# georgegrosu1/torch-admm-deconv

Hardware: AMD Instinct MI355X
Metric: ADMM iterations/sec, batch-64 1024x1024x3, 50 iters; rel-L2 vs CPU ref (higher is better)
Workload: dtype f32

## Files before the change

### torch-admm-deconv_amd/csrc/admm_capi.hip

```cpp
#include <hip/hip_runtime.h>

#include <cstdlib>
#include <cstring>
#include <mutex>
#include <string>
#include <type_traits>
#include <vector>

#include "gcol_mm.hpp"
#include "knobs.hpp"
#include "mixed_capi.hpp"
#include "odd_capi.hpp"
#include "state_kernels.hpp"
#include "admm_tv.h"

using namespace admm;

namespace {

thread_local std::string g_err;

int fail(int code, const std::string& msg) {
    g_err = msg;
    return code;
// ... 88 lines not shown
    size_t lds;
    int nth;
};
MMPlan mm_plan(int H, int W);
MMPlan mm_plan_row(int W);

int ngroups_of(const admm_tv_desc& d) { return d.groups > 1 ? d.groups : 1; }

bool is_bank(const admm_tv_desc& d) { return (d.flags & (ADMM_TV_FLAG_PSF_PER_IMAGE | ADMM_TV_FLAG_PSF_PER_CHANNEL)) != 0; }
BankIdx bank_of(const admm_tv_desc& d) {
    const int Bk = (d.flags & ADMM_TV_FLAG_PSF_PER_IMAGE) ? (int)d.B : 1;
    const int Ck = (d.flags & ADMM_TV_FLAG_PSF_PER_CHANNEL) ? (int)d.C : 1;
    return BankIdx{(int)d.C, Bk > 1 ? Ck : 0, Ck > 1 ? 1 : 0, Bk * Ck};
}
int bank_run(const admm_tv_desc& d) { return (d.flags & ADMM_TV_FLAG_PSF_PER_CHANNEL) ? 1 : (int)d.C; }
constexpr long long kBankMax = 65535;

constexpr size_t kAlign = 256;
size_t up(size_t v) { return (v + kAlign - 1) / kAlign * kAlign; }

struct Layout {
    size_t spec[2], u[4], b, fcT, mT, twW, twH, twHd, G, part, nsq, sigma, total;
    size_t mM;
    MMPlan mm, mmr;
    bool mixed, mixed_train;
    size_t fcM;
    bool odd;
    size_t spec2;
    bool tr;
    size_t xT, oT, kT, tws;
    size_t rimg;
    size_t gscr;
    int ngroups, ppg;
    bool gen;
    int ldw;
};

admm_tv_desc transposed(const admm_tv_desc& d) {
    admm_tv_desc t = d;
    t.H = d.W;
    t.W = d.H;
    t.kh = d.kw;
    t.kw = d.kh;
    return t;
}

// ... 15 lines not shown
    size_t o = 0;
    auto take = [&](size_t bytes) {
        size_t at = o;
        o += up(bytes);
        return at;
    };
    L.gen = f64 || generic_hw(d.H, d.W);
    if (L.gen && !f64) {
        if (!bank) L.mm = mm_plan((int)H, (int)W);
        L.mmr = mm_plan_row((int)W);
    }
    L.mixed = L.gen && !f64 && mixed_hw(d.H, d.W) && (G == 1 || !(d.flags & ADMM_TV_FLAG_PSF_GRAD));
    L.mixed_train = mixed_train_hw(d);
    L.odd = L.gen && !f64 && G == 1 && !d.iso && !bank && odd_hw(d.H, d.W);
    L.ldw = (int)(N + 1);
    if (L.gen && !f64 && L.mm.ok && L.mmr.ok && env_int("ADMM_GEN_PITCH", 1)) L.ldw = (int)((N + 1 + 15) / 16 * 16);
    L.spec[0] = take(L.gen ? P * H * (size_t)L.ldw * csz : img);
    L.spec[1] = take(img);
    L.rimg = L.gen ? take(img) : 0;
    for (int i = 0; i < 4; ++i) L.u[i] = take(img);
    L.b = (k > 0 || !L.gen) ? take(img_m) : 0;
    L.fcT = take(G * T * (N + 1) * H * rs * ((!L.gen || L.mm.ok) ? 2 : 1));
    L.mT = take(T * (N + 1) * H * csz);
    L.twW = take((W + (L.gen ? make_plan((int)W, f64).ntab : 0)) * csz);
    L.twH = take((H + (L.gen ? make_plan((int)H, f64).ntab : 0)) * csz);
    L.twHd = take(H * sizeof(double2));
    L.G = take(T * (size_t)(k > 0 ? k : 1) * (N + 1) * sizeof(double2));
    L.gscr = L.gen ? take(glb_scratch((int)H, (int)W, (long long)P, f64)) : 0;
    L.fcM = L.mixed ? take(G * T * (2 * N + 1) * H * sizeof(float)) : 0;
    L.mM = (L.mixed && k > 0) ? take(T * (N + 1) * H * 2 * sizeof(float)) : 0;
    L.spec2 = L.odd ? take(P * H * (size_t)L.ldw * csz) : 0;
    L.sigma = (k > 0 && (d.flags & ADMM_TV_FLAG_PSF_GRAD)) ? take((N + 1) * H * sizeof(double2)) : 0;
    if (d.iso) {
        const int lanes = (int)std::min<size_t>(64, N / (N >= 1024 ? 16 : N >= 64 ? 8 : N >= 16 ? 4 : 2));
        const long long want = 3LL * 1024 * 64 / std::max(lanes, 1);
        int ppg = (int)std::max<long long>(1, std::min<long long>(64, (long long)(P * H) / want));
        if (const int e = env_int("ADMM_ISO_PPG", 0); e > 0) ppg = e;
        if ((size_t)P <= (size_t)ppg) ppg = (int)std::max<long long>(1, P);
        if (G > 1) {
            const int pm = (int)(d.B * d.C);
            ppg = std::min(ppg, pm);
            while (pm % ppg) --ppg;
        }
        L.ppg = ppg;
        L.ngroups = (int)((P + ppg - 1) / ppg);
        L.part = take((size_t)L.ngroups * 2 * H * W * rs);
// ... 46 lines not shown
}

int check_workspace(const void* ws, size_t have, size_t need) {
    if (!ws || have < need || (reinterpret_cast<uintptr_t>(ws) % kAlign) != 0)
        return fail(ADMM_TV_EWORKSPACE, "workspace too small or not 256-byte aligned");
    return 0;
}

template <class T>
int bwd_scalars(double* part, int K, long long nstrips, long long spm, long long soff, const double* tpart, int ntp,
                int G, int g, const T* lam, const T* rho, T* glam, T* grho, hipStream_t s) {
    if (K < 1) return fail(ADMM_TV_EINVAL, "bwd_scalars: no iterations");
    hipLaunchKernelGGL(k_bwd_iter_sums, dim3((unsigned)K), dim3(256), 0, s, part, nstrips, spm, soff, tpart, ntp, G, g);
    if (int e = launch_check("k_bwd_iter_sums")) return e;
    hipLaunchKernelGGL(k_bwd_scalars<T>, dim3(1), dim3(256), 0, s, (const double*)part, K, nstrips, 1LL, soff,
                       (const double*)nullptr, ntp, G, g, lam, rho, glam, grho);
    return launch_check("k_bwd_scalars");
}

template <int N> struct RowOps {
    using G = RowKernelGeom<N>;
    static unsigned blocks(long long items) { return (unsigned)((items + G::SG - 1) / G::SG); }

    static int r2c(const float* img, cf* spec, const cf* twW, long long rows, hipStream_t s, bool pl = false) {
        if (pl)
            hipLaunchKernelGGL((k_row_r2c<N, true>), dim3(blocks(rows)), dim3(G::NT), G::lds_bytes(), s, img, spec, twW, rows);
        else
            hipLaunchKernelGGL((k_row_r2c<N, false>), dim3(blocks(rows)), dim3(G::NT), G::lds_bytes(), s, img, spec, twW, rows);
        return launch_check("k_row_r2c");
    }
    static int c2r(const cf* spec, float* img, const cf* twW, long long rows, hipStream_t s, bool pl = false) {
        if (pl)
            hipLaunchKernelGGL((k_row_c2r<N, true>), dim3(blocks(rows)), dim3(G::NT), G::lds_bytes(), s, spec, img, twW, rows);
        else
            hipLaunchKernelGGL((k_row_c2r<N, false>), dim3(blocks(rows)), dim3(G::NT), G::lds_bytes(), s, spec, img, twW, rows);
        return launch_check("k_row_c2r");
    }
    static int pair(const float* img, float* out, long long rows, hipStream_t s) {
        hipLaunchKernelGGL(k_row_pair<N>, dim3(blocks(rows)), dim3(G::NT), 0, s, img, out, rows);
        return launch_check("k_row_pair");
    }
    template <bool ISO, bool FIRST, bool HIST, bool PL> static void pa(const PassAArgs& a, unsigned nb, hipStream_t s) {
        hipLaunchKernelGGL((k_pass_a<N, ISO, FIRST, HIST, PL>), dim3(nb), dim3(G::NT), G::lds_bytes(), s, a);
    }
    static constexpr bool kCoop = N == 512;
    template <bool FIRST, bool PL> static void pa_coop(const PassAArgs& a, unsigned nb, hipStream_t s, bool pf) {
        if constexpr (kCoop) {
            if (pf)
                hipLaunchKernelGGL((k_pass_a<N, false, FIRST, false, PL, true, true>), dim3(nb), dim3(G::NT), passa_coop_lds<N>(), s, a);
            else
                hipLaunchKernelGGL((k_pass_a<N, false, FIRST, false, PL, true>), dim3(nb), dim3(G::NT), passa_coop_lds<N>(), s, a);
        }
    }
    static int pass_a(const PassAArgs& a, bool iso, bool first, bool hist, hipStream_t s, bool pl = false,
                      bool coop = false, bool pf = false) {
// ... 94 lines not shown
        case 256: return f(std::integral_constant<int, 256>{});
        case 512: return f(std::integral_constant<int, 512>{});
        case 1024: return f(std::integral_constant<int, 1024>{});
        case 2048: return f(std::integral_constant<int, 2048>{});
        case 4096: return f(std::integral_constant<int, 4096>{});
        default: return fail(ADMM_TV_EUNSUPPORTED, "unsupported H");
    }
}

int col_e(int H) { return H >= 1024 ? 16 : H >= 64 ? 8 : 4; }

int passb_order(int H) { return std::max(1, std::min(64, env_int("ADMM_PASSB_GROUP", H >= 1024 ? 2 : 1))); }

int passb_gp(int H, int P, int ppm) {
    (void)H;
    int g = env_int("ADMM_PASSB_GP", 1);
    g = std::max(1, std::min(g, 64));
    while (g > 1 && (ppm % g)) --g;
    (void)P;
    return g;
}

template <int H, int C> int pass_b_hc(const cf* spec, cf* out, const float* fcT, const cf* mT, const cf* twH, int N,
                                      int P, int mode, int ppm, hipStream_t s, const BankIdx* bank) {
    using G = ColGeom<H, C>;
    const int colblocks = N / C;
    const int gp = passb_gp(H, P, ppm);
    const dim3 grid((unsigned)((long long)((P + gp - 1) / gp) * colblocks));
    const int order = gp > 1 ? 1 : passb_order(H);
    const int fpack = mode == 0 && env_int("ADMM_PASSB_FPACK", 1) ? 1 : 0;
    const int pmode = env_int("ADMM_PASSB_PMODE", 2);
    if (bank) {
        if (mode == 0) {
            if (int e = set_lds(k_pass_b<H, C, 0, BankIdx>, G::lds_bytes())) return e;
            hipLaunchKernelGGL((k_pass_b<H, C, 0, BankIdx>), grid, dim3(G::NT), G::lds_bytes(), s, spec, out, fcT, mT, twH, N,
                               colblocks, ppm, order, fpack, gp, P, pmode, *bank);
        } else if (mode == 1) {
            if (int e = set_lds(k_pass_b<H, C, 1, BankIdx>, G::lds_bytes())) return e;
            hipLaunchKernelGGL((k_pass_b<H, C, 1, BankIdx>), grid, dim3(G::NT), G::lds_bytes(), s, spec, out, fcT, mT, twH, N,
                               colblocks, ppm, order, fpack, gp, P, pmode, *bank);
        } else {
            return fail(ADMM_TV_EUNSUPPORTED, "PSF bank: no adjoint column pass (inference only)");
        }
        return launch_check("k_pass_b<bank>");
    }
    if (mode == 0) {
        if (int e = set_lds(k_pass_b<H, C, 0>, G::lds_bytes())) return e;
        hipLaunchKernelGGL((k_pass_b<H, C, 0>), grid, dim3(G::NT), G::lds_bytes(), s, spec, out, fcT, mT, twH, N, colblocks, ppm,
                           order, fpack, gp, P, pmode);
    } else if (mode == 1) {
        if (int e = set_lds(k_pass_b<H, C, 1>, G::lds_bytes())) return e;
        hipLaunchKernelGGL((k_pass_b<H, C, 1>), grid, dim3(G::NT), G::lds_bytes(), s, spec, out, fcT, mT, twH, N, colblocks, ppm,
                           order, fpack, gp, P, pmode);
    } else {
        if (int e = set_lds(k_pass_b<H, C, 2>, G::lds_bytes())) return e;
        hipLaunchKernelGGL((k_pass_b<H, C, 2>), grid, dim3(G::NT), G::lds_bytes(), s, spec, out, fcT, mT, twH, N, colblocks, ppm,
                           order, fpack, gp, P, pmode);
    }
    return launch_check("k_pass_b");
}

template <int H> int pass_b_h(const cf* spec, cf* out, const float* fcT, const cf* mT, const cf* twH, int N, int P,
                              int mode, int ppm, hipStream_t s, const BankIdx* bank) {
    constexpr int L = ColGeom<H, 1>::L;
    if constexpr (L <= 64) {
        if (mode == 0 && N >= 16 && env_int("ADMM_PASSB_PAIR", H <= 512 ? 1 : 0)) {
            using G = ColGeom<H, 8>;
            const int colblocks = N / 16;
            if (bank) {
                if (int e = set_lds(k_pass_b2<H, 8, BankIdx>, G::lds_bytes())) return e;
                hipLaunchKernelGGL((k_pass_b2<H, 8, BankIdx>), dim3((unsigned)((long long)P * colblocks)), dim3(G::NT),
                                   G::lds_bytes(), s, spec, out, fcT, twH, N, colblocks, ppm, passb_order(H),
                                   env_int("ADMM_PASSB_FPACK", 1) ? 1 : 0, *bank);
                return launch_check("k_pass_b2<bank>");
            }
            if (int e = set_lds(k_pass_b2<H, 8>, G::lds_bytes())) return e;
            hipLaunchKernelGGL((k_pass_b2<H, 8>), dim3((unsigned)((long long)P * colblocks)), dim3(G::NT), G::lds_bytes(),
                               s, spec, out, fcT, twH, N, colblocks, ppm, passb_order(H), env_int("ADMM_PASSB_FPACK", 1) ? 1 : 0);
            return launch_check("k_pass_b2");
        }
        int C = env_int("ADMM_PASSB_C", 8);
        if (C > N) C = N;
        if (C >= 16) return pass_b_hc<H, 16>(spec, out, fcT, mT, twH, N, P, mode, ppm, s, bank);
        return pass_b_hc<H, 8>(spec, out, fcT, mT, twH, N, P, mode, ppm, s, bank);
    } else if constexpr (L == 128) {
        return pass_b_hc<H, 8>(spec, out, fcT, mT, twH, N, P, mode, ppm, s, bank);
    } else {
        return pass_b_hc<H, 4>(spec, out, fcT, mT, twH, N, P, mode, ppm, s, bank);
    }
}

int pass_b_oop(int H, const cf* spec, cf* out, const float* fcT, const cf* mT, const cf* twH, int N, int P, int mode,
               hipStream_t s, int ppm = 0, const BankIdx* bank = nullptr) {
    if (ppm <= 0) ppm = P;
    return with_col(H, [&](auto h) { return pass_b_h<decltype(h)::value>(spec, out, fcT, mT, twH, N, P, mode, ppm, s, bank); });
}

int pass_b(int H, cf* spec, const float* fcT, const cf* mT, const cf* twH, int N, int P, int mode, hipStream_t s,
           int ppm = 0, const BankIdx* bank = nullptr) {
    return pass_b_oop(H, spec, spec, fcT, mT, twH, N, P, mode, s, ppm, bank);
}

template <int H, int C> int xspec_hc(const cf* U, const cf* V, cf* part, const cf* twH, int N, int P, int ppg,
                                     hipStream_t s) {
    using G = ColGeom<H, C>;
    const int colblocks = N / C;
    const int groups = (P + ppg - 1) / ppg;
    if (int e = set_lds(k_xspec<H, C, true>, G::lds_bytes())) return e;
    if (int e = set_lds(k_xspec<H, C, false>, G::lds_bytes())) return e;
    hipLaunchKernelGGL((k_xspec<H, C, true>), dim3(groups), dim3(G::NT), G::lds_bytes(), s, U, V, part, twH, N,
                       colblocks, P, ppg);
    if (colblocks > 1)
        hipLaunchKernelGGL((k_xspec<H, C, false>), dim3(groups * (colblocks - 1)), dim3(G::NT), G::lds_bytes(), s, U,
                           V, part, twH, N, colblocks, P, ppg);
    return launch_check("k_xspec");
}
template <int H> int xspec_h(const cf* U, const cf* V, cf* part, const cf* twH, int N, int P, int ppg, hipStream_t s) {
    constexpr int L = ColGeom<H, 1>::L;
    if constexpr (L <= 64) return xspec_hc<H, 8>(U, V, part, twH, N, P, ppg, s);
    else if constexpr (L == 128) return xspec_hc<H, 8>(U, V, part, twH, N, P, ppg, s);
    else return xspec_hc<H, 4>(U, V, part, twH, N, P, ppg, s);
}
int xspec(int H, const cf* U, const cf* V, cf* part, const cf* twH, int N, int P, int ppg, hipStream_t s) {
// ... 20 lines not shown
    if (d->groups > 1 && ((!supported_hw(d->H, d->W) && !mixed_hw(d->H, d->W)) || (d->flags & ADMM_TV_FLAG_PSF_GRAD)))
        return fail(ADMM_TV_EUNSUPPORTED, "groups > 1 needs power-of-two or smooth H, W and no PSF gradient");
    return 0;
}

int bank_check(const admm_tv_desc& d, bool train = false, bool f64 = false) {
    if (!is_bank(d)) return 0;
    if (f64 || is_f64(d)) return fail(ADMM_TV_EUNSUPPORTED, "PSF bank: fp32 only (ADMM_TV_FLAG_F64 / an _f64 entry point)");
    if (train) return fail(ADMM_TV_EUNSUPPORTED, "PSF bank: inference only (training with a bank is not implemented)");
    if (d.flags & ADMM_TV_FLAG_PSF_GRAD) return fail(ADMM_TV_EUNSUPPORTED, "PSF bank: no PSF gradient (ADMM_TV_FLAG_PSF_GRAD)");
    if (d.kh == 0) return fail(ADMM_TV_EINVAL, "PSF bank without a PSF (kh == 0)");
    if (d.groups > 1) return fail(ADMM_TV_EUNSUPPORTED, "PSF bank: groups > 1 (one solve per module)");
    if (d.allreduce) return fail(ADMM_TV_EUNSUPPORTED, "PSF bank: no cross-rank all-reduce hook");
    const long long T = ((d.flags & ADMM_TV_FLAG_PSF_PER_IMAGE) ? d.B : 1) * ((d.flags & ADMM_TV_FLAG_PSF_PER_CHANNEL) ? d.C : 1);
    if (T > kBankMax || d.B > 0x7fffffffLL || d.C > 0x7fffffffLL)
        return fail(ADMM_TV_EUNSUPPORTED, "PSF bank: more than 65,535 PSFs");
    return 0;
}

double spectra_scale(int H, int W) {
    return (supported_hw(H, W) ? 0.5 : 1.0) / ((double)H * (double)W);
}

int bank_spectra(const admm_tv_desc& d, const Layout& Lo, void* ws, const float* rho, float* fcT, hipStream_t s) {
    const int H = (int)d.H, W = (int)d.W, N = W / 2, nt = 256, n = (N + 1) * H;
    const unsigned T = (unsigned)bank_of(d).T;
    hipLaunchKernelGGL(k_spectra_bank, dim3((n + nt - 1) / nt, T), dim3(nt), 0, s, at<double2>(ws, Lo.G),
                       at<double2>(ws, Lo.twHd), rho, fcT, at<cf>(ws, Lo.mT), d.kh, H, N, W, spectra_scale(H, W));
    if (int e = launch_check("k_spectra_bank")) return e;
    if (Lo.mixed) return hip_code(admm_mixed::mt_mixed(at<cf>(ws, Lo.mT), at<cf>(ws, Lo.mM), H, N, s, (int)T), "k_mt_mixed_bank");
    return 0;
}
int setup_bank(const admm_tv_desc& d, const Layout& Lo, void* ws, const float* kern, const float* rho, hipStream_t s) {
    const int H = (int)d.H, W = (int)d.W, N = W / 2, k = d.kh, nt = 256, n = (N + 1) * H;
    const unsigned T = (unsigned)bank_of(d).T;
    hipLaunchKernelGGL(k_psf_rows_bank, dim3((k * (N + 1) + nt - 1) / nt, T), dim3(nt), 0, s, kern, at<double2>(ws, Lo.G), k,
                       N, W);
    if (int e = launch_check("k_psf_rows_bank")) return e;
    if (!rho) return 0;
    float* fc = at<float>(ws, Lo.fcT);
    if (int e = bank_spectra(d, Lo, ws, rho, fc, s)) return e;
    if (!Lo.gen) {
        hipLaunchKernelGGL(k_fc_pack_bank, dim3((n + nt - 1) / nt, T), dim3(nt), 0, s, fc, fc + (size_t)T * n, H, N, col_e(H));
        if (int e = launch_check("k_fc_pack_bank")) return e;
    }
    if (Lo.mixed) return hip_code(admm_mixed::fc_mixed(fc, at<float>(ws, Lo.fcM), H, N, s, (int)T), "k_fc_mixed_bank");
    return 0;
}

template <class T>
int setup(const admm_tv_desc& d, const Layout& Lo, void* ws, const T* kern, const T* rho, hipStream_t s) {
    using C = cx_t<T>;
// ... 27 lines not shown
                               at<double2>(ws, Lo.twHd), rho + g, at<T>(ws, Lo.fcT) + (size_t)g * n, at<C>(ws, Lo.mT),
                               k, H, N, W, Lo.sigma ? at<double2>(ws, Lo.sigma) : nullptr,
                               (std::is_same<T, double>::value ? 1.0 / ((double)H * W) : spectra_scale(H, W)));
            if (int e = launch_check("k_spectra")) return e;
            if constexpr (std::is_same<T, float>::value) if (!Lo.gen) {
                float* fc = at<float>(ws, Lo.fcT) + (size_t)g * n;
                hipLaunchKernelGGL(k_fc_pack, dim3((n + nt - 1) / nt), dim3(nt), 0, s, fc,
                                   fc + (size_t)ngroups_of(d) * n, H, N, col_e(H));
                if (int e = launch_check("k_fc_pack")) return e;
            }
            if constexpr (std::is_same<T, float>::value) if (Lo.mixed) {
                if (int e = hip_code(admm_mixed::fc_mixed(at<float>(ws, Lo.fcT) + (size_t)g * n,
                                                          at<float>(ws, Lo.fcM) + (size_t)g * (2 * N + 1) * H, H, N, s),
                                     "k_fc_mixed"))
                    return e;
            }
            if constexpr (std::is_same<T, float>::value) if (Lo.gen && Lo.mm.ok && ngroups_of(d) == 1) {
                float* fc = at<float>(ws, Lo.fcT);
                hipLaunchKernelGGL(k_fc_transpose, dim3(std::min(4096, (n + nt - 1) / nt)), dim3(nt), 0, s, fc, fc + n, H,
                                   N + 1);
                if (int e = launch_check("k_fc_transpose")) return e;
            }
        }
        if constexpr (std::is_same<T, float>::value) if (Lo.mixed && k > 0) {
            if (int e = hip_code(admm_mixed::mt_mixed(at<cf>(ws, Lo.mT), at<cf>(ws, Lo.mM), H, N, s), "k_mt_mixed")) return e;
        }
    }
    return 0;
}

int pow2_floor(int v);

int strip_rows(int H, int N, long long rows, bool aniso_fwd = false, bool coop = false) {
    int R = env_int("ADMM_PASSA_R", 0);
    if (R > 0) R = pow2_floor(std::max(2, std::min(R, H)));
    if (R <= 0) {
        const int L = std::min(64, N / (N >= 1024 ? 16 : N >= 64 ? 8 : N >= 16 ? 4 : 2));
        long long want = 3LL * 1024 * 64 / L;
        R = 8;
        if (aniso_fwd && N == 256) {
            R = 16;
            want /= 2;
        }
        if (coop && aniso_fwd && N == 512 && (H / 4) % 4 == 0) R = 4;
        while (R > 2 && rows / R < want) R /= 2;
    }
// ... 78 lines not shown
            hipError_t e = hipEventRecord(joins[i], aux[i]);
            if (e == hipSuccess) e = hipStreamWaitEvent(s, joins[i], 0);
            if (first == hipSuccess) first = e;
        }
        return first;
    }
    ~ForkJoin() {
        if (fork) (void)hipEventDestroy(fork);
        for (hipEvent_t j : joins)
            if (j) (void)hipEventDestroy(j);
    }
};

std::vector<long long> gen_parts(long long P, int H, int ns) {
    long long c = (P + ns - 1) / std::max(ns, 1);
    if (H & 1) c += c & 1;
    std::vector<long long> starts;
    for (long long p = 0; p < P; p += std::max(c, 1LL)) starts.push_back(p);
    return starts;
}


int psf_transpose_into(const admm_tv_desc& d, const Layout& Lo, void* ws, const float* xin, float* bb, cf* spec,
                       int mode, hipStream_t s, bool pl = false) {
    const long long rows = d.B * d.C * d.H;
    const int H = (int)d.H, N = (int)d.W / 2;
    cf* twW = at<cf>(ws, Lo.twW);
    int e = with_row(N, [&](auto ops) { return decltype(ops)::r2c(xin, spec, twW, rows, s); });
    if (e) return e;
    const BankIdx bk = bank_of(d);
    if ((e = pass_b(H, spec, at<float>(ws, Lo.fcT), at<cf>(ws, Lo.mT), at<cf>(ws, Lo.twH), N, (int)(d.B * d.C), mode, s,
                    is_bank(d) ? bank_run(d) : 0, is_bank(d) ? &bk : nullptr)))
        return e;
    return with_row(N, [&](auto ops) { return decltype(ops)::c2r(spec, bb, twW, rows, s, pl); });
}


GPlan make_plan_radices(int n);

int blue_min() { return env_int("ADMM_BLUE_MIN", 41); }

constexpr size_t kMaxLds = 160 * 1024;
size_t glds(int n, int lines, const GPlan& p, size_t csz = sizeof(cf)) {
    if (p.glb) return 0;
    return csz * ((p.twg ? 0 : (size_t)n + p.ntab) + 2 * (size_t)n * lines + p.xslots);
}

constexpr long long kGlbSlots = 1024;
constexpr size_t kGlbBudget = 512ull << 20;
long long glb_slots(int n, size_t csz) {
    return std::max<long long>(64, std::min<long long>(kGlbSlots, (long long)(kGlbBudget / (2 * (size_t)n * csz))));
}

GPlan make_plan_f64(int n) {
    GPlan p{};
    p.n = n;
    int m = n, r = n;
// ... 853 lines not shown
    FusedOps(const admm_tv_desc& d_, const Layout& L, void* w)
        : d(d_), Lo(L), ws(w), H((int)d_.H), N((int)d_.W / 2), twW(at<cf>(w, L.twW)), twH(at<cf>(w, L.twH)) {}
};

struct Pow2Ops : FusedOps {
    static constexpr bool kPsfGrad = true;
    float* const fcT;
    cf* const mT;
    const bool coop;
    const int rev;
    const bool pf;
    Pow2Ops(const admm_tv_desc& d_, const Layout& L, void* w)
        : FusedOps(d_, L, w), fcT(at<float>(w, L.fcT)), mT(at<cf>(w, L.mT)),
          coop(env_int("ADMM_PASSA_COOP", 1) != 0), rev(env_int("ADMM_PASSA_REV", 0)),
          pf(env_int("ADMM_PASSA_PF", 1) != 0) {}
    int modules_per_pass(int G) const { return G; }
    bool lane_paired(bool train) const { return !train && env_int("ADMM_PL", (d.iso || d.W < 1024) ? 1 : 0) != 0; }
    int row_lanes() const {
        int L = 0;
        with_row(N, [&](auto ops) { return L = decltype(ops)::G::L; });
        return L;
    }
    int strip(long long rows, bool aniso_fwd) const { return strip_rows(H, N, rows, aniso_fwd, coop && !rev); }
    int r2c(const float* img, cf* spec, long long rows, hipStream_t s, bool pl = false) const {
        return with_row(N, [&](auto ops) { return decltype(ops)::r2c(img, spec, twW, rows, s, pl); });
    }
    int c2r(const cf* spec, float* img, long long rows, hipStream_t s) const {
        return with_row(N, [&](auto ops) { return decltype(ops)::c2r(spec, img, twW, rows, s); });
    }
    int col(const cf* in, cf* out, long long np, long long ppm, int , hipStream_t s) const {
        if (is_bank(d)) {
            const BankIdx bk = bank_of(d);
            return pass_b_oop(H, in, out, fcT, mT, twH, N, (int)np, 0, s, bank_run(d), &bk);
        }
        return pass_b_oop(H, in, out, fcT, mT, twH, N, (int)np, 0, s, (int)ppm);
    }
    int xspec(const cf* U, const cf* V, cf* part, long long P, int ppg, bool , hipStream_t s) const {
        return ::xspec(H, U, V, part, twH, N, (int)P, ppg, s);
    }
    int iso_norm(const IsoArgs& a, bool first, bool hist, hipStream_t s, bool pl) const {
        return with_row(N, [&](auto ops) { return decltype(ops)::iso_norm(a, first, hist, s, pl); });
    }
    int pass_a(const PassAArgs& a, bool iso, bool first, bool hist, hipStream_t s, bool pl) const {
        return with_row(N, [&](auto ops) { return decltype(ops)::pass_a(a, iso, first, hist, s, pl, coop, pf); });
    }
    int bwd_iso_q(const BwdIsoArgs& a, bool lastk, hipStream_t s) const {
        return with_row(N, [&](auto ops) { return decltype(ops)::bwd_iso_q(a, lastk, s); });
    }
    int bwd_pass_a(const BwdArgs& a, bool iso, bool lastk, bool firstk, hipStream_t s) const {
        return with_row(N, [&](auto ops) { return decltype(ops)::bwd_pass_a(a, iso, lastk, firstk, s); });
    }
    int make_b(const float* xin, float* bb, cf* spec, bool pl, hipStream_t s) const {
        if (d.kh > 0) return psf_transpose_into(d, Lo, ws, xin, bb, spec, 1, s, pl);
        return with_row(N, [&](auto ops) { return decltype(ops)::pair(xin, bb, d.B * d.C * H, s); });
    }
    int apply_ht_t(const float* bbar, float* gxin, cf* spec, hipStream_t s) const {
        return psf_transpose_into(d, Lo, ws, bbar, gxin, spec, 2, s);
    }
};

struct MixedOps : FusedOps {
    static constexpr bool kPsfGrad = true;
    const float* const fcM;
    static constexpr int rev = 0;
    MixedOps(const admm_tv_desc& d_, const Layout& L, void* w) : FusedOps(d_, L, w), fcM(at<float>(w, L.fcM)) {}
    int modules_per_pass(int) const { return 1; }
    bool lane_paired(bool) const { return false; }
    int row_lanes() const { return 0; }
    int strip(long long rows, bool) const { return strip_rows_mixed(H, rows, N); }
    int r2c(const float* img, cf* spec, long long rows, hipStream_t s, bool = false) const {
        return hip_code(admm_mixed::r2c(N, img, spec, twW, rows, s), "k_row_r2c_m");
    }
    int c2r(const cf* spec, float* img, long long rows, hipStream_t s) const {
        return hip_code(admm_mixed::c2r(N, spec, img, twW, rows, s), "k_row_c2r_m");
    }
    int col(const cf* in, cf* out, long long np, long long, int g0, hipStream_t s) const {
        if (is_bank(d)) {
            const BankIdx bk = bank_of(d);
            return hip_code(admm_mixed::pass_b(H, in, out, fcM, twH, N, np, s, &bk), "k_pass_b_m<bank>");
        }
        return hip_code(admm_mixed::pass_b(H, in, out, fcM + (size_t)g0 * (2 * N + 1) * H, twH, N, np, s), "k_pass_b_m");
    }
    int xspec(const cf* U, const cf* V, cf* part, long long P, int ppg, bool weighted, hipStream_t s) const {
        return hip_code(admm_mixed::xspec(H, U, V, part, twH, N, P, ppg, weighted ? 0.25f : 1.f, s), "k_xspec_m");
    }
    int iso_norm(const IsoArgs& a, bool first, bool hist, hipStream_t s, bool) const {
        return hip_code(admm_mixed::iso_norm(N, a, first, hist, s), "k_iso_norm_m");
    }
    int pass_a(const PassAArgs& a, bool iso, bool first, bool hist, hipStream_t s, bool) const {
        return hip_code(admm_mixed::pass_a(N, a, iso, first, hist, s), "k_pass_a_m");
    }
    int bwd_iso_q(const BwdIsoArgs& a, bool lastk, hipStream_t s) const {
        return hip_code(admm_mixed::bwd_iso_q(N, a, lastk, s), "k_bwd_iso_q_m");
    }
    int bwd_pass_a(const BwdArgs& a, bool iso, bool lastk, bool firstk, hipStream_t s) const {
        return hip_code(admm_mixed::bwd_pass_a(N, a, iso, lastk, firstk, s), "k_bwd_pass_a_m");
    }
    int make_b(const float* xin, float* bb, cf* spec, bool, hipStream_t s) const {
        const long long P = d.B * d.C;
        if (env_int("ADMM_MIXED_BGEN", 0)) return gapply<float>(xin, bb, spec, Lo, ws, d, 1, s);
        if (int e = r2c(xin, spec, P * H, s)) return e;
        const BankIdx bk = bank_of(d);
        if (int e = hip_code(admm_mixed::pass_b_cm(H, spec, at<cf>(ws, Lo.mM), twH, N, P, s, is_bank(d) ? &bk : nullptr),
                             "k_pass_b_m<cm>"))
            return e;
        return c2r(spec, bb, P * H, s);
    }
    int apply_ht_t(const float* bbar, float* gxin, cf* spec, hipStream_t s) const {
        return gapply<float>(bbar, gxin, spec, Lo, ws, d, 2, s);
    }
};

template <class B>
int fused_forward(const B& be, const float* xin, const float* lam, const float* rho, float* out, void* hist,
                  hipStream_t s, const StateIO* sio = nullptr) {
    const admm_tv_desc& d = be.d;
    const Layout& Lo = be.Lo;
    void* ws = be.ws;
    const int H = be.H, N = be.N, W = (int)d.W, G = ngroups_of(d);
    const long long Pm = d.B * d.C;
    cf* spec[2] = {at<cf>(ws, Lo.spec[0]), at<cf>(ws, Lo.spec[1])};
    float* u[4] = {at<float>(ws, Lo.u[0]), at<float>(ws, Lo.u[1]), at<float>(ws, Lo.u[2]), at<float>(ws, Lo.u[3])};
    const bool train = hist != nullptr;
    const HistView<float> hv(d, hist);
    const bool keep_t = B::kPsfGrad && train && hv.h.keep_t;
    const bool pl = be.lane_paired(train);
    const float* bimg = xin;
    if (d.kh > 0 || pl) {
        ProfScope ps(3, s);
        float* bb = at<float>(ws, Lo.b);
        if (int e = be.make_b(xin, bb, spec[0], pl, s)) return e;
        bimg = bb;
    }
    const int ng = be.modules_per_pass(G);
    const long long np = ng * Pm, rows = np * H;
    const int gpm = Lo.ngroups / G;
    const int R = be.strip(rows, !d.iso && !train);
    const bool sin = sio && sio->in, sout = sio && sio->out;
    const int sl = pl ? be.row_lanes() : 0;
    for (int g0 = 0; g0 < G; g0 += ng) {
        const float* lamg = lam + g0;
        const float* rhog = rho + g0;
        float* outg = out + (size_t)g0 * Pm * H * W;
        for (int g = 0; g < ng; ++g) {
            ProfScope ps(3, s);
            cf* t0 = (keep_t ? hv.r(1) : spec[0]) + (size_t)g * Pm * H * N;
            if (sin) {
                if (int e = state_import(d, *sio->in, bimg, outg, u[0], u[1], lamg, rhog, sl, s)) return e;
                if (int e = be.r2c(outg, t0, Pm * H, s, false)) return e;
                continue;
            }
            if (int e = be.r2c(bimg, t0, Pm * H, s, pl)) return e;
        }
        int cur = 0, uin = 0;
        for (int it = 1; it <= d.maxit; ++it) {
            {
                ProfScope ps(1, s);
                if (int e = be.col(keep_t ? hv.r(it) : spec[cur], spec[cur], np, Pm, g0, s)) return e;
            }
            if (it == d.maxit) {
                ProfScope ps(3, s);
                if (int e = be.c2r(spec[cur], outg, rows, s)) return e;
                if (sout) {
                    const bool none = d.maxit == 1 && !sin;
                    if (int e = state_export(d, Lo, ws, outg, none ? nullptr : u[2 * uin], none ? nullptr : u[2 * uin + 1],
                                             *sio->out, lamg, rhog, sl, s))
                        return e;
                }
                if (!train) break;
// ... 599 lines not shown
    DeviceGuard dg(reinterpret_cast<hipStream_t>(stream));
    if (int e = dg.check()) return e;
    const Layout Lo = make_layout(d);
    if (!ws || ws_bytes < Lo.total) return fail(ADMM_TV_EWORKSPACE, "workspace too small");
    const long long P = d.B * d.C;
    const int H = (int)d.H, W = (int)d.W, N = W / 2;
    if (d.kh == 0) {
        HIPCHK(hipMemcpyAsync(out, xin, (size_t)P * H * W * sizeof(float), hipMemcpyDeviceToDevice, s));
        return 0;
    }
    if (int e = setup<float>(d, Lo, ws, kern, nullptr, s)) return e;
    const int n = (N + 1) * H;
    HIPCHK(hipMemsetAsync(at<float>(ws, Lo.fcT), 0, sizeof(float), s));
    if (is_bank(d)) {
        if (int e = bank_spectra(d, Lo, ws, at<float>(ws, Lo.fcT), at<float>(ws, Lo.spec[1]), s)) return e;
        if (Lo.mixed) return MixedOps(d, Lo, ws).make_b(xin, out, at<cf>(ws, Lo.spec[0]), false, s);
        if (Lo.gen) return gapply(xin, out, at<cf>(ws, Lo.spec[0]), Lo, ws, d, 1, s);
        return psf_transpose_into(d, Lo, ws, xin, out, at<cf>(ws, Lo.spec[0]), 1, s);
    }
    hipLaunchKernelGGL(k_spectra<float>, dim3((n + 255) / 256), dim3(256), 0, s, at<double2>(ws, Lo.G),
                       at<double2>(ws, Lo.twHd), at<float>(ws, Lo.fcT), at<float>(ws, Lo.spec[1]),
                       at<cf>(ws, Lo.mT), d.kh, H, N, W, nullptr, spectra_scale(H, W));
    if (int e = launch_check("k_spectra")) return e;
    if (Lo.gen) return gapply(xin, out, at<cf>(ws, Lo.spec[0]), Lo, ws, d, 1, s);
    return psf_transpose_into(d, Lo, ws, xin, out, at<cf>(ws, Lo.spec[0]), 1, s);
}

int admm_tv_forward_f64(const admm_tv_desc* dp, const double* xin, const double* kern, const double* lam,
                        const double* rho, double* out, void* ws, size_t ws_bytes, void* stream) {
    if (int e = validate(dp)) return e;
    if (int e = bank_check(*dp, false, true)) return e;
    if (!is_f64(*dp)) return fail(ADMM_TV_EINVAL, "admm_tv_forward_f64 needs ADMM_TV_FLAG_F64");
    if (((!xin || !out) && !participate_only(*dp)) || !lam || !rho || (dp->kh > 0 && !kern))
        return fail(ADMM_TV_EINVAL, "null pointer argument");
    DeviceGuard dg(reinterpret_cast<hipStream_t>(stream));
    if (int e = dg.check()) return e;
    return run_forward_f64(*dp, xin, kern, lam, rho, out, ws, ws_bytes, nullptr, reinterpret_cast<hipStream_t>(stream));
}

int admm_tv_forward_train_f64(const admm_tv_desc* dp, const double* xin, const double* kern, const double* lam,
                              const double* rho, double* out, void* hist, size_t hist_bytes, void* ws, size_t ws_bytes,
                              void* stream) {
    if (int e = validate(dp)) return e;
    if (int e = bank_check(*dp, false, true)) return e;
    if (!is_f64(*dp)) return fail(ADMM_TV_EINVAL, "admm_tv_forward_train_f64 needs ADMM_TV_FLAG_F64");
    if (((!xin || !out) && !participate_only(*dp)) || !lam || !rho || (dp->kh > 0 && !kern))
// ... 66 lines not shown
```

### torch-admm-deconv_amd/csrc/admm_kernels.hpp

```cpp
#pragma once
#include "fft_core.hpp"

namespace admm {

template <int N, class Cfg = RowCfg<N>> struct RowXf {
    static constexpr int E = Cfg::E;
    static constexpr int L = N / E;
    static constexpr int W = 2 * N;
    static_assert(L <= 64, "row transforms keep one row inside one wave");

    __device__ __forceinline__ static void partner(const cf (&v)[E], cf (&p)[E], int t) {
        const int src = (L - t) & (L - 1);
#pragma unroll
        for (int j = 0; j < E; ++j) {
            float a = __shfl(v[E - 1 - j].x, src, L);
            float b = __shfl(v[E - 1 - j].y, src, L);
            p[j] = (t == 0) ? v[(E - j) & (E - 1)] : mkc(a, b);
        }
    }

    template <int SYNC = 0>
    __device__ __forceinline__ static void c2r(cf (&v)[E], const RowBuf& buf, const cf* __restrict__ tw, int t) {
        cf p[E];
        partner(v, p, t);
// ... 206 lines not shown
            const f4v q = __builtin_bit_cast(f4v, __builtin_amdgcn_raw_buffer_load_b128(r, voff + L * j * 16, soff, AUX));
            v[2 * j] = mkc(q.x, q.y);
            v[2 * j + 1] = mkc(q.z, q.w);
        }
    } else {
#pragma unroll
        for (int j = 0; j < E; ++j) v[j] = bload_cf<AUX>(r, voff + L * j * 8, soff);
    }
}
template <int E, int L, bool PL, int AUX> __device__ __forceinline__ void bst_row(rsrc_t r, int voff, int soff, const cf (&v)[E]) {
    if constexpr (PL) {
        typedef decltype(__builtin_amdgcn_raw_buffer_load_b128(r, 0, 0, 0)) V4;
#pragma unroll
        for (int j = 0; j < E / 2; ++j) {
            const f4v q = {v[2 * j].x, v[2 * j].y, v[2 * j + 1].x, v[2 * j + 1].y};
            __builtin_amdgcn_raw_buffer_store_b128(__builtin_bit_cast(V4, q), r, voff + L * j * 16, soff, AUX);
        }
    } else {
#pragma unroll
        for (int j = 0; j < E; ++j) bstore_cf<AUX>(r, voff + L * j * 8, soff, v[j]);
    }
}

template <int N, bool PL>
__global__ void __launch_bounds__(256) k_row_r2c(const float* __restrict__ img, cf* __restrict__ spec,
                                                 const cf* __restrict__ twW_g, long long rows) {
    using G = RowKernelGeom<N>;
    constexpr int E = G::E, L = G::L;
    extern __shared__ __attribute__((aligned(16))) unsigned char smem[];
    cf* tw = reinterpret_cast<cf*>(smem);
    load_tw(tw, twW_g, G::W);
    __syncthreads();
    const int sgl = threadIdx.x / L, t = threadIdx.x % L;
    const long long row = (long long)blockIdx.x * G::SG + sgl;
    if (row >= rows) return;
    RowBuf buf{tw + G::W + sgl * RowBuf::slots(N)};
    const cf* src = reinterpret_cast<const cf*>(img + row * G::W);
    cf v[E];
    ld_row<E, L, PL, false>(src, t, v);
    RowXf<N>::r2c(v, buf, tw, t);
    cf* dst = spec + row * N;
#pragma unroll
    for (int j = 0; j < E; ++j) dst[t + L * j] = v[j];
}

template <int N, bool PL>
__global__ void __launch_bounds__(256) k_row_c2r(const cf* __restrict__ spec, float* __restrict__ img,
                                                 const cf* __restrict__ twW_g, long long rows) {
    using G = RowKernelGeom<N>;
    constexpr int E = G::E, L = G::L;
    extern __shared__ __attribute__((aligned(16))) unsigned char smem[];
    cf* tw = reinterpret_cast<cf*>(smem);
    load_tw(tw, twW_g, G::W);
    __syncthreads();
    const int sgl = threadIdx.x / L, t = threadIdx.x % L;
    const long long row = (long long)blockIdx.x * G::SG + sgl;
    if (row >= rows) return;
    RowBuf buf{tw + G::W + sgl * RowBuf::slots(N)};
    const cf* src = spec + row * N;
    cf v[E];
#pragma unroll
    for (int j = 0; j < E; ++j) v[j] = src[t + L * j];
    RowXf<N>::c2r(v, buf, tw, t);
    cf* dst = reinterpret_cast<cf*>(img + row * G::W);
    st_row<E, L, PL, false>(dst, t, v);
}

template <int N>
__global__ void __launch_bounds__(256) k_row_pair(const float* __restrict__ img, float* __restrict__ out, long long rows) {
    using G = RowKernelGeom<N>;
    constexpr int E = G::E, L = G::L;
    const int sgl = threadIdx.x / L, t = threadIdx.x % L;
    const long long row = (long long)blockIdx.x * G::SG + sgl;
    if (row >= rows) return;
    cf v[E];
    ld_row<E, L, false, true>(reinterpret_cast<const cf*>(img + row * G::W), t, v);
    st_row<E, L, true, false>(reinterpret_cast<cf*>(out + row * G::W), t, v);
}

constexpr int pb_minw(int nt, size_t lds) {
    return (nt / 64 * ((160 * 1024) / lds >= 2 ? 2 : 1) + 3) / 4 > 4 ? 4
                                                                      : (nt / 64 * ((160 * 1024) / lds >= 2 ? 2 : 1) + 3) / 4;
}

template <int H, int C> struct ColGeom {
    static constexpr int E = RowCfg<H>::E, L = H / E, NT = C * L;
    static constexpr int SYNC = 1;
    static constexpr size_t lds_bytes() { return sizeof(cf) * (H + (size_t)H * C); }
};

static __global__ void k_fc_pack(const float* __restrict__ fcT, float* __restrict__ fcP, int H, int N, int E) {
    const int i = blockIdx.x * blockDim.x + threadIdx.x;
    if (i >= (N + 1) * H) return;
    const int L = H / E, kx = i / H, r = i % H, t = r / E, j = r % E;
    fcP[i] = fcT[(size_t)kx * H + t + L * j];
}
static __global__ void k_fc_pack_bank(const float* __restrict__ fcT, float* __restrict__ fcP, int H, int N, int E) {
    const int i = blockIdx.x * blockDim.x + threadIdx.x;
    if (i >= (N + 1) * H) return;
    const size_t o = (size_t)blockIdx.y * (N + 1) * H;
    const int L = H / E, kx = i / H, r = i % H, t = r / E, j = r % E;
    fcP[o + i] = fcT[o + (size_t)kx * H + t + L * j];
}

__device__ __forceinline__ unsigned xcd_remap(unsigned b, unsigned nb) {
    const unsigned x = b & 7u, i = b >> 3, q = nb >> 3, r = nb & 7u;
    return (x < r ? x * (q + 1) : r * (q + 1) + (x - r) * q) + i;
}

__device__ __forceinline__ unsigned xcd_pairs(unsigned b, unsigned nb) {
    if ((b | 15u) >= nb) return b;
    const unsigned x = b & 7u, s = b >> 3;
    return 2u * (8u * (s >> 1) + x) + (s & 1u);
}

__device__ __forceinline__ void pb_tile(unsigned lb, int colblocks, int order, bool pairs, int& p, int& cb) {
    const unsigned P = gridDim.x / (unsigned)colblocks, G = order > 1 ? (unsigned)order : 1u;
    const unsigned per = G * (unsigned)colblocks, grp = lb / per;
    if (G == 1 || (pairs && (colblocks & 1)) || (grp + 1) * G > P) {
        p = (int)(lb / (unsigned)colblocks);
        cb = (int)(lb % (unsigned)colblocks);
        return;
    }
    const unsigned rem = lb % per;
    if (pairs) {
// ... 13 lines not shown
__global__ void __launch_bounds__(C * (H / RowCfg<H>::E), pb_minw(C * (H / RowCfg<H>::E), sizeof(cf) * (H + (size_t)H * C)))
    k_pass_b(const cf* spec_in, cf* spec_out, const float* __restrict__ fcT, const cf* __restrict__ mT,
             const cf* __restrict__ twH_g, int N, int colblocks, int ppm, int order, int fpack, int gp, int P,
             int pmode, BK... bk) {
    constexpr bool BANK = sizeof...(BK) > 0;
    using G = ColGeom<H, C>;
    constexpr int E = G::E, L = G::L;
    extern __shared__ __attribute__((aligned(16))) unsigned char smem[];
    cf* tw = reinterpret_cast<cf*>(smem);
    cf* data = tw + H;
    load_tw(tw, twH_g, H);
    const int tid = threadIdx.x;
    const int c = tid % C, t = tid / C;
    const unsigned rb = (pmode >> 1) == 1 ? xcd_remap(blockIdx.x, gridDim.x)
                        : (pmode >> 1) == 2 ? xcd_pairs(blockIdx.x, gridDim.x) : blockIdx.x;
    int pg, cb;
    pb_tile(rb, colblocks, order, true, pg, cb);
    if (pmode & 1) pg = (int)(gridDim.x / (unsigned)colblocks) - 1 - pg;
    const int col = cb * C + c;
    const int p0 = pg * gp;
    if constexpr (BANK) {
        const size_t to = (size_t)bank_tab(p0, bk...) * (N + 1) * H;
        if (MODE == 0) fcT += to;
        else mT += to;
    } else {
        if (MODE == 0) fcT += (size_t)(p0 / ppm) * (N + 1) * H;
    }
    const int voff = (t * N + col) * (int)sizeof(cf);
    const int sstep = L * N * (int)sizeof(cf);
    using MT = typename std::conditional<MODE == 0, float, cf>::type;
    MT m[E];
    auto load_m = [&]() {
        if (MODE == 0 && fpack) {
            const float* fcP = fcT + (size_t)bank_tables(P / ppm, bk...) * (N + 1) * H;
            const float4* qq = reinterpret_cast<const float4*>(fcP + ((size_t)col * L + t) * E);
    #pragma unroll
            for (int j = 0; j < E / 4; ++j) {
                const float4 f = qq[j];
                if constexpr (MODE == 0) {
                    m[4 * j] = f.x;
                    m[4 * j + 1] = f.y;
                    m[4 * j + 2] = f.z;
                    m[4 * j + 3] = f.w;
                }
            }
        } else {
            const rsrc_t rm = MODE == 0 ? make_rsrc(fcT, (unsigned)((size_t)(N + 1) * H * sizeof(float)))
                                        : make_rsrc(mT, (unsigned)((size_t)(N + 1) * H * sizeof(cf)));
            const int mo = (col * H + t) * (int)sizeof(MT);
    #pragma unroll
            for (int j = 0; j < E; ++j) {
                if constexpr (MODE == 0) m[j] = bload_f(rm, mo, j * L * (int)sizeof(float));
                else if constexpr (MODE == 1) m[j] = bload_cf(rm, mo, j * L * (int)sizeof(cf));
                else m[j] = cconj(bload_cf(rm, mo, j * L * (int)sizeof(cf)));
            }
        }
// ... 686 lines not shown
```

Before: 744.0.

## Pack adjoint PSF spectrum for vector loads and reuse b-spectrum as first iterate

```diff
diff --git a/torch-admm-deconv_amd/csrc/admm_capi.hip b/torch-admm-deconv_amd/csrc/admm_capi.hip
--- a/torch-admm-deconv_amd/csrc/admm_capi.hip
+++ b/torch-admm-deconv_amd/csrc/admm_capi.hip
@@ -134,6 +134,7 @@
 struct Layout {
     size_t spec[2], u[4], b, fcT, mT, twW, twH, twHd, G, part, nsq, sigma, total;
     size_t mM;
+    size_t mP;
     MMPlan mm, mmr;
     bool mixed, mixed_train;
     size_t fcM;
@@ -195,6 +196,7 @@
     L.b = (k > 0 || !L.gen) ? take(img_m) : 0;
     L.fcT = take(G * T * (N + 1) * H * rs * ((!L.gen || L.mm.ok) ? 2 : 1));
     L.mT = take(T * (N + 1) * H * csz);
+    L.mP = (k > 0 && !L.gen) ? take(T * (N + 1) * H * csz) : 0;
     L.twW = take((W + (L.gen ? make_plan((int)W, f64).ntab : 0)) * csz);
     L.twH = take((H + (L.gen ? make_plan((int)H, f64).ntab : 0)) * csz);
     L.twHd = take(H * sizeof(double2));
@@ -287,15 +289,24 @@
     using G = RowKernelGeom<N>;
     static unsigned blocks(long long items) { return (unsigned)((items + G::SG - 1) / G::SG); }
 
-    static int r2c(const float* img, cf* spec, const cf* twW, long long rows, hipStream_t s, bool pl = false) {
-        if (pl)
+    static int r2c(const float* img, cf* spec, const cf* twW, long long rows, hipStream_t s, bool pl = false,
+                   bool sc = false) {
+        if (sc && pl) return fail(ADMM_TV_EINVAL, "k_row_r2c: the scaled transform reads pixel-order rows");
+        if (sc)
+            hipLaunchKernelGGL((k_row_r2c<N, false, true>), dim3(blocks(rows)), dim3(G::NT), G::lds_bytes(), s, img, spec, twW, rows);
+        else if (pl)
             hipLaunchKernelGGL((k_row_r2c<N, true>), dim3(blocks(rows)), dim3(G::NT), G::lds_bytes(), s, img, spec, twW, rows);
         else
             hipLaunchKernelGGL((k_row_r2c<N, false>), dim3(blocks(rows)), dim3(G::NT), G::lds_bytes(), s, img, spec, twW, rows);
         return launch_check("k_row_r2c");
     }
-    static int c2r(const cf* spec, float* img, const cf* twW, long long rows, hipStream_t s, bool pl = false) {
-        if (pl)
+    static int c2r(const cf* spec, float* img, const cf* twW, long long rows, hipStream_t s, bool pl = false,
+                   bool sc = false) {
+        if (sc && pl)
+            hipLaunchKernelGGL((k_row_c2r<N, true, true>), dim3(blocks(rows)), dim3(G::NT), G::lds_bytes(), s, spec, img, twW, rows);
+        else if (sc)
+            hipLaunchKernelGGL((k_row_c2r<N, false, true>), dim3(blocks(rows)), dim3(G::NT), G::lds_bytes(), s, spec, img, twW, rows);
+        else if (pl)
             hipLaunchKernelGGL((k_row_c2r<N, true>), dim3(blocks(rows)), dim3(G::NT), G::lds_bytes(), s, spec, img, twW, rows);
         else
             hipLaunchKernelGGL((k_row_c2r<N, false>), dim3(blocks(rows)), dim3(G::NT), G::lds_bytes(), s, spec, img, twW, rows);
@@ -436,13 +447,15 @@
 }
 
 template <int H, int C> int pass_b_hc(const cf* spec, cf* out, const float* fcT, const cf* mT, const cf* twH, int N,
-                                      int P, int mode, int ppm, hipStream_t s, const BankIdx* bank) {
+                                      int P, int mode, int ppm, hipStream_t s, const BankIdx* bank, const cf* mP) {
     using G = ColGeom<H, C>;
     const int colblocks = N / C;
     const int gp = passb_gp(H, P, ppm);
     const dim3 grid((unsigned)((long long)((P + gp - 1) / gp) * colblocks));
     const int order = gp > 1 ? 1 : passb_order(H);
-    const int fpack = mode == 0 && env_int("ADMM_PASSB_FPACK", 1) ? 1 : 0;
+    const bool mpack = mode != 0 && mP && env_int("ADMM_PASSB_MPACK", 1);
+    const int fpack = (mode == 0 && env_int("ADMM_PASSB_FPACK", 1)) || mpack ? 1 : 0;
+    const float* fm = mpack ? reinterpret_cast<const float*>(mP) : fcT;
     const int pmode = env_int("ADMM_PASSB_PMODE", 2);
     if (bank) {
         if (mode == 0) {
@@ -451,7 +464,7 @@
                                colblocks, ppm, order, fpack, gp, P, pmode, *bank);
         } else if (mode == 1) {
             if (int e = set_lds(k_pass_b<H, C, 1, BankIdx>, G::lds_bytes())) return e;
-            hipLaunchKernelGGL((k_pass_b<H, C, 1, BankIdx>), grid, dim3(G::NT), G::lds_bytes(), s, spec, out, fcT, mT, twH, N,
+            hipLaunchKernelGGL((k_pass_b<H, C, 1, BankIdx>), grid, dim3(G::NT), G::lds_bytes(), s, spec, out, fm, mT, twH, N,
                                colblocks, ppm, order, fpack, gp, P, pmode, *bank);
         } else {
             return fail(ADMM_TV_EUNSUPPORTED, "PSF bank: no adjoint column pass (inference only)");
@@ -464,18 +477,18 @@
                            order, fpack, gp, P, pmode);
     } else if (mode == 1) {
         if (int e = set_lds(k_pass_b<H, C, 1>, G::lds_bytes())) return e;
-        hipLaunchKernelGGL((k_pass_b<H, C, 1>), grid, dim3(G::NT), G::lds_bytes(), s, spec, out, fcT, mT, twH, N, colblocks, ppm,
+        hipLaunchKernelGGL((k_pass_b<H, C, 1>), grid, dim3(G::NT), G::lds_bytes(), s, spec, out, fm, mT, twH, N, colblocks, ppm,
                            order, fpack, gp, P, pmode);
     } else {
         if (int e = set_lds(k_pass_b<H, C, 2>, G::lds_bytes())) return e;
-        hipLaunchKernelGGL((k_pass_b<H, C, 2>), grid, dim3(G::NT), G::lds_bytes(), s, spec, out, fcT, mT, twH, N, colblocks, ppm,
+        hipLaunchKernelGGL((k_pass_b<H, C, 2>), grid, dim3(G::NT), G::lds_bytes(), s, spec, out, fm, mT, twH, N, colblocks, ppm,
                            order, fpack, gp, P, pmode);
     }
     return launch_check("k_pass_b");
 }
 
 template <int H> int pass_b_h(const cf* spec, cf* out, const float* fcT, const cf* mT, const cf* twH, int N, int P,
-                              int mode, int ppm, hipStream_t s, const BankIdx* bank) {
+                              int mode, int ppm, hipStream_t s, const BankIdx* bank, const cf* mP) {
     constexpr int L = ColGeom<H, 1>::L;
     if constexpr (L <= 64) {
         if (mode == 0 && N >= 16 && env_int("ADMM_PASSB_PAIR", H <= 512 ? 1 : 0)) {
@@ -495,24 +508,24 @@
         }
         int C = env_int("ADMM_PASSB_C", 8);
         if (C > N) C = N;
-        if (C >= 16) return pass_b_hc<H, 16>(spec, out, fcT, mT, twH, N, P, mode, ppm, s, bank);
-        return pass_b_hc<H, 8>(spec, out, fcT, mT, twH, N, P, mode, ppm, s, bank);
+        if (C >= 16) return pass_b_hc<H, 16>(spec, out, fcT, mT, twH, N, P, mode, ppm, s, bank, mP);
+        return pass_b_hc<H, 8>(spec, out, fcT, mT, twH, N, P, mode, ppm, s, bank, mP);
     } else if constexpr (L == 128) {
-        return pass_b_hc<H, 8>(spec, out, fcT, mT, twH, N, P, mode, ppm, s, bank);
+        return pass_b_hc<H, 8>(spec, out, fcT, mT, twH, N, P, mode, ppm, s, bank, mP);
     } else {
-        return pass_b_hc<H, 4>(spec, out, fcT, mT, twH, N, P, mode, ppm, s, bank);
+        return pass_b_hc<H, 4>(spec, out, fcT, mT, twH, N, P, mode, ppm, s, bank, mP);
     }
 }
 
 int pass_b_oop(int H, const cf* spec, cf* out, const float* fcT, const cf* mT, const cf* twH, int N, int P, int mode,
-               hipStream_t s, int ppm = 0, const BankIdx* bank = nullptr) {
+               hipStream_t s, int ppm = 0, const BankIdx* bank = nullptr, const cf* mP = nullptr) {
     if (ppm <= 0) ppm = P;
-    return with_col(H, [&](auto h) { return pass_b_h<decltype(h)::value>(spec, out, fcT, mT, twH, N, P, mode, ppm, s, bank); });
+    return with_col(H, [&](auto h) { return pass_b_h<decltype(h)::value>(spec, out, fcT, mT, twH, N, P, mode, ppm, s, bank, mP); });
 }
 
 int pass_b(int H, cf* spec, const float* fcT, const cf* mT, const cf* twH, int N, int P, int mode, hipStream_t s,
-           int ppm = 0, const BankIdx* bank = nullptr) {
-    return pass_b_oop(H, spec, spec, fcT, mT, twH, N, P, mode, s, ppm, bank);
+           int ppm = 0, const BankIdx* bank = nullptr, const cf* mP = nullptr) {
+    return pass_b_oop(H, spec, spec, fcT, mT, twH, N, P, mode, s, ppm, bank, mP);
 }
 
 template <int H, int C> int xspec_hc(const cf* U, const cf* V, cf* part, const cf* twH, int N, int P, int ppg,
@@ -579,12 +592,14 @@
     return (supported_hw(H, W) ? 0.5 : 1.0) / ((double)H * (double)W);
 }
 
+int mt_pack(const admm_tv_desc& d, const Layout& Lo, void* ws, hipStream_t s);
 int bank_spectra(const admm_tv_desc& d, const Layout& Lo, void* ws, const float* rho, float* fcT, hipStream_t s) {
     const int H = (int)d.H, W = (int)d.W, N = W / 2, nt = 256, n = (N + 1) * H;
     const unsigned T = (unsigned)bank_of(d).T;
     hipLaunchKernelGGL(k_spectra_bank, dim3((n + nt - 1) / nt, T), dim3(nt), 0, s, at<double2>(ws, Lo.G),
                        at<double2>(ws, Lo.twHd), rho, fcT, at<cf>(ws, Lo.mT), d.kh, H, N, W, spectra_scale(H, W));
     if (int e = launch_check("k_spectra_bank")) return e;
+    if (int e = mt_pack(d, Lo, ws, s)) return e;
     if (Lo.mixed) return hip_code(admm_mixed::mt_mixed(at<cf>(ws, Lo.mT), at<cf>(ws, Lo.mM), H, N, s, (int)T), "k_mt_mixed_bank");
     return 0;
 }
@@ -658,6 +673,9 @@
                 if (int e = launch_check("k_fc_transpose")) return e;
             }
         }
+        if constexpr (std::is_same<T, float>::value) if (k > 0) {
+            if (int e = mt_pack(d, Lo, ws, s)) return e;
+        }
         if constexpr (std::is_same<T, float>::value) if (Lo.mixed && k > 0) {
             if (int e = hip_code(admm_mixed::mt_mixed(at<cf>(ws, Lo.mT), at<cf>(ws, Lo.mM), H, N, s), "k_mt_mixed")) return e;
         }
@@ -782,17 +800,25 @@
 
 
 int psf_transpose_into(const admm_tv_desc& d, const Layout& Lo, void* ws, const float* xin, float* bb, cf* spec,
-                       int mode, hipStream_t s, bool pl = false) {
+                       int mode, hipStream_t s, bool pl = false, bool r1 = false) {
     const long long rows = d.B * d.C * d.H;
     const int H = (int)d.H, N = (int)d.W / 2;
     cf* twW = at<cf>(ws, Lo.twW);
-    int e = with_row(N, [&](auto ops) { return decltype(ops)::r2c(xin, spec, twW, rows, s); });
+    int e = with_row(N, [&](auto ops) { return decltype(ops)::r2c(xin, spec, twW, rows, s, false, r1); });
     if (e) return e;
     const BankIdx bk = bank_of(d);
     if ((e = pass_b(H, spec, at<float>(ws, Lo.fcT), at<cf>(ws, Lo.mT), at<cf>(ws, Lo.twH), N, (int)(d.B * d.C), mode, s,
-                    is_bank(d) ? bank_run(d) : 0, is_bank(d) ? &bk : nullptr)))
+                    is_bank(d) ? bank_run(d) : 0, is_bank(d) ? &bk : nullptr, Lo.mP ? at<cf>(ws, Lo.mP) : nullptr)))
         return e;
-    return with_row(N, [&](auto ops) { return decltype(ops)::c2r(spec, bb, twW, rows, s, pl); });
+    return with_row(N, [&](auto ops) { return decltype(ops)::c2r(spec, bb, twW, rows, s, pl, r1); });
+}
+
+int mt_pack(const admm_tv_desc& d, const Layout& Lo, void* ws, hipStream_t s) {
+    if (!Lo.mP) return 0;
+    const int H = (int)d.H, N = (int)d.W / 2, nt = 256, n = (N + 1) * H;
+    const unsigned T = is_bank(d) ? (unsigned)bank_of(d).T : 1u;
+    hipLaunchKernelGGL(k_mt_pack, dim3((n + nt - 1) / nt, T), dim3(nt), 0, s, at<cf>(ws, Lo.mT), at<cf>(ws, Lo.mP), H, N, col_e(H));
+    return launch_check("k_mt_pack");
 }
 
 
@@ -1692,6 +1718,10 @@
         return L;
     }
     int strip(long long rows, bool aniso_fwd) const { return strip_rows(H, N, rows, aniso_fwd, coop && !rev); }
+    bool r1_from_b() const {
+        const int k = env_int("ADMM_R1_REUSE", 1);
+        return d.kh > 0 && (k >= 2 || (k == 1 && !d.iso));
+    }
     int r2c(const float* img, cf* spec, long long rows, hipStream_t s, bool pl = false) const {
         return with_row(N, [&](auto ops) { return decltype(ops)::r2c(img, spec, twW, rows, s, pl); });
     }
@@ -1720,8 +1750,8 @@
     int bwd_pass_a(const BwdArgs& a, bool iso, bool lastk, bool firstk, hipStream_t s) const {
         return with_row(N, [&](auto ops) { return decltype(ops)::bwd_pass_a(a, iso, lastk, firstk, s); });
     }
-    int make_b(const float* xin, float* bb, cf* spec, bool pl, hipStream_t s) const {
-        if (d.kh > 0) return psf_transpose_into(d, Lo, ws, xin, bb, spec, 1, s, pl);
+    int make_b(const float* xin, float* bb, cf* spec, bool pl, hipStream_t s, bool r1 = false) const {
+        if (d.kh > 0) return psf_transpose_into(d, Lo, ws, xin, bb, spec, 1, s, pl, r1);
         return with_row(N, [&](auto ops) { return decltype(ops)::pair(xin, bb, d.B * d.C * H, s); });
     }
     int apply_ht_t(const float* bbar, float* gxin, cf* spec, hipStream_t s) const {
@@ -1738,6 +1768,7 @@
     bool lane_paired(bool) const { return false; }
     int row_lanes() const { return 0; }
     int strip(long long rows, bool) const { return strip_rows_mixed(H, rows, N); }
+    bool r1_from_b() const { return false; }
     int r2c(const float* img, cf* spec, long long rows, hipStream_t s, bool = false) const {
         return hip_code(admm_mixed::r2c(N, img, spec, twW, rows, s), "k_row_r2c_m");
     }
@@ -1766,7 +1797,7 @@
     int bwd_pass_a(const BwdArgs& a, bool iso, bool lastk, bool firstk, hipStream_t s) const {
         return hip_code(admm_mixed::bwd_pass_a(N, a, iso, lastk, firstk, s), "k_bwd_pass_a_m");
     }
-    int make_b(const float* xin, float* bb, cf* spec, bool, hipStream_t s) const {
+    int make_b(const float* xin, float* bb, cf* spec, bool, hipStream_t s, bool = false) const {
         const long long P = d.B * d.C;
         if (env_int("ADMM_MIXED_BGEN", 0)) return gapply<float>(xin, bb, spec, Lo, ws, d, 1, s);
         if (int e = r2c(xin, spec, P * H, s)) return e;
@@ -1795,18 +1826,20 @@
     const HistView<float> hv(d, hist);
     const bool keep_t = B::kPsfGrad && train && hv.h.keep_t;
     const bool pl = be.lane_paired(train);
+    const bool sin = sio && sio->in, sout = sio && sio->out;
+    const bool r1b = be.r1_from_b() && !sin;
+    cf* const r1 = keep_t ? hv.r(1) : spec[0];
     const float* bimg = xin;
     if (d.kh > 0 || pl) {
         ProfScope ps(3, s);
         float* bb = at<float>(ws, Lo.b);
-        if (int e = be.make_b(xin, bb, spec[0], pl, s)) return e;
+        if (int e = be.make_b(xin, bb, r1b ? r1 : spec[0], pl, s, r1b)) return e;
         bimg = bb;
     }
     const int ng = be.modules_per_pass(G);
     const long long np = ng * Pm, rows = np * H;
     const int gpm = Lo.ngroups / G;
     const int R = be.strip(rows, !d.iso && !train);
-    const bool sin = sio && sio->in, sout = sio && sio->out;
     const int sl = pl ? be.row_lanes() : 0;
     for (int g0 = 0; g0 < G; g0 += ng) {
         const float* lamg = lam + g0;
@@ -1814,7 +1847,11 @@
         float* outg = out + (size_t)g0 * Pm * H * W;
         for (int g = 0; g < ng; ++g) {
             ProfScope ps(3, s);
-            cf* t0 = (keep_t ? hv.r(1) : spec[0]) + (size_t)g * Pm * H * N;
+            cf* t0 = r1 + (size_t)g * Pm * H * N;
+            if (r1b) {
+                if (g > 0) HIPCHK(hipMemcpyAsync(t0, r1, (size_t)Pm * H * N * sizeof(cf), hipMemcpyDeviceToDevice, s));
+                continue;
+            }
             if (sin) {
                 if (int e = state_import(d, *sio->in, bimg, outg, u[0], u[1], lamg, rhog, sl, s)) return e;
                 if (int e = be.r2c(outg, t0, Pm * H, s, false)) return e;
@@ -2460,6 +2497,7 @@
                        at<double2>(ws, Lo.twHd), at<float>(ws, Lo.fcT), at<float>(ws, Lo.spec[1]),
                        at<cf>(ws, Lo.mT), d.kh, H, N, W, nullptr, spectra_scale(H, W));
     if (int e = launch_check("k_spectra")) return e;
+    if (int e = mt_pack(d, Lo, ws, s)) return e;
     if (Lo.gen) return gapply(xin, out, at<cf>(ws, Lo.spec[0]), Lo, ws, d, 1, s);
     return psf_transpose_into(d, Lo, ws, xin, out, at<cf>(ws, Lo.spec[0]), 1, s);
 }
diff --git a/torch-admm-deconv_amd/csrc/admm_kernels.hpp b/torch-admm-deconv_amd/csrc/admm_kernels.hpp
--- a/torch-admm-deconv_amd/csrc/admm_kernels.hpp
+++ b/torch-admm-deconv_amd/csrc/admm_kernels.hpp
@@ -252,7 +252,7 @@
     }
 }
 
-template <int N, bool PL>
+template <int N, bool PL, bool SC = false>
 __global__ void __launch_bounds__(256) k_row_r2c(const float* __restrict__ img, cf* __restrict__ spec,
                                                  const cf* __restrict__ twW_g, long long rows) {
     using G = RowKernelGeom<N>;
@@ -270,11 +270,15 @@
     ld_row<E, L, PL, false>(src, t, v);
     RowXf<N>::r2c(v, buf, tw, t);
     cf* dst = spec + row * N;
+    if constexpr (SC) {
+#pragma unroll
+        for (int j = 0; j < E; ++j) v[j] = cscale(v[j], (float)(2 * G::W));
+    }
 #pragma unroll
     for (int j = 0; j < E; ++j) dst[t + L * j] = v[j];
 }
 
-template <int N, bool PL>
+template <int N, bool PL, bool SC = false>
 __global__ void __launch_bounds__(256) k_row_c2r(const cf* __restrict__ spec, float* __restrict__ img,
                                                  const cf* __restrict__ twW_g, long long rows) {
     using G = RowKernelGeom<N>;
@@ -292,6 +296,10 @@
 #pragma unroll
     for (int j = 0; j < E; ++j) v[j] = src[t + L * j];
     RowXf<N>::c2r(v, buf, tw, t);
+    if constexpr (SC) {
+#pragma unroll
+        for (int j = 0; j < E; ++j) v[j] = cscale(v[j], 1.f / (float)(2 * G::W));
+    }
     cf* dst = reinterpret_cast<cf*>(img + row * G::W);
     st_row<E, L, PL, false>(dst, t, v);
 }
@@ -331,6 +339,14 @@
     const size_t o = (size_t)blockIdx.y * (N + 1) * H;
     const int L = H / E, kx = i / H, r = i % H, t = r / E, j = r % E;
     fcP[o + i] = fcT[o + (size_t)kx * H + t + L * j];
+}
+
+static __global__ void k_mt_pack(const cf* __restrict__ mT, cf* __restrict__ mP, int H, int N, int E) {
+    const int i = blockIdx.x * blockDim.x + threadIdx.x;
+    if (i >= (N + 1) * H) return;
+    const size_t o = (size_t)blockIdx.y * (N + 1) * H;
+    const int L = H / E, kx = i / H, r = i % H, t = r / E, j = r % E;
+    mP[o + i] = mT[o + (size_t)kx * H + t + L * j];
 }
 
 __device__ __forceinline__ unsigned xcd_remap(unsigned b, unsigned nb) {
@@ -390,7 +406,10 @@
     if constexpr (BANK) {
         const size_t to = (size_t)bank_tab(p0, bk...) * (N + 1) * H;
         if (MODE == 0) fcT += to;
-        else mT += to;
+        else {
+            mT += to;
+            fcT += 2 * to;
+        }
     } else {
         if (MODE == 0) fcT += (size_t)(p0 / ppm) * (N + 1) * H;
     }
@@ -399,7 +418,20 @@
     using MT = typename std::conditional<MODE == 0, float, cf>::type;
     MT m[E];
     auto load_m = [&]() {
-        if (MODE == 0 && fpack) {
+        if (MODE != 0 && fpack) {
+            const float4* qq = reinterpret_cast<const float4*>(fcT) + ((size_t)col * L + t) * (E / 2);
+    #pragma unroll
+            for (int j = 0; j < E / 2; ++j) {
+                const float4 f = qq[j];
+                if constexpr (MODE == 1) {
+                    m[2 * j] = mkc(f.x, f.y);
+                    m[2 * j + 1] = mkc(f.z, f.w);
+                } else if constexpr (MODE == 2) {
+                    m[2 * j] = cconj(mkc(f.x, f.y));
+                    m[2 * j + 1] = cconj(mkc(f.z, f.w));
+                }
+            }
+        } else if (MODE == 0 && fpack) {
             const float* fcP = fcT + (size_t)bank_tables(P / ppm, bk...) * (N + 1) * H;
             const float4* qq = reinterpret_cast<const float4*>(fcP + ((size_t)col * L + t) * E);
     #pragma unroll
```

Result: no change. 747.3 (median of 6 runs) (+0.4%).
